# wwood/CoverM

Measured on NVIDIA H100. Metric: reads/sec `coverm contig` (mean+trimmed_mean+covered_fraction), higher is better.
Workload: dtype i32

## Files before the change

coverm_b200/csrc/cmb_k2.cuh:

```cuda
#pragma once
#include "cmb_k2_slots.cuh"

struct K2Args {
  const uint32_t* off_span;
  const uint32_t* len;
  const uint32_t* chunk_first;
  const int32_t* carry_in;
  cmb_contig_stats* rows;
  uint32_t tid_begin, n_local, n_chunks, excl;
  int32_t* arena;
  const uint32_t* word_off;
  const uint16_t* buckets;
  uint32_t* span_bits;
  uint32_t* load_stats;
  const uint64_t* bin_base;
  uint32_t* bins;
  uint64_t pool_cap;
  uint32_t* bin_hi;
  uint32_t* error_flags;
};

#ifndef CMB_K2_DENSE_SPANS
#define CMB_K2_DENSE_SPANS 160
#endif
constexpr uint32_t K2_DENSE_SPANS = CMB_K2_DENSE_SPANS;
static_assert(K2_STAGES >= 2, "a round's rows are requested one round before it is reduced");
static_assert(K2_CHUNK_SPANS == CHUNK_SPANS && K2_WARPS == 8, "a chunk is 8 bitmap words of 32 spans");

constexpr uint32_t K2_ROUND = 32;
constexpr uint32_t K2_BUF_BYTES = K2_ROUND * 128;
constexpr uint32_t K2_BOX_ROWS = K2_ROUND;
constexpr uint32_t K2_STAGE_CODES = 1024;
constexpr uint32_t K2_STAGE_BYTES = K2_STAGE_CODES * 2;
template <bool BUCKETS>
__host__ __device__ constexpr uint32_t k2_warp_bytes() { return BUCKETS ? K2_BUF_BYTES + K2_STAGES * K2_STAGE_BYTES : K2_STAGES * K2_BUF_BYTES; }
constexpr uint32_t K2_CHUNK_CONTIGS = 16;
struct K2ChunkContigs {
  uint64_t bin[K2_CHUNK_CONTIGS + 1];
  uint32_t start[K2_CHUNK_CONTIGS];
  uint32_t len[K2_CHUNK_CONTIGS];
};
struct K2WarpTables {
  K2ChunkContigs ct;
  uint8_t span[2][K2_CHUNK_SPANS];
  uint8_t pre[2][8];
};
static_assert(sizeof(K2WarpTables) % 8 == 0, "the contig tables hold u64 bins");
constexpr uint32_t K2_SMEM_MISC = K2_WARPS * K2_STAGES * 8  +
                                  K2_WARPS * 128  +
                                  K2_WARPS * sizeof(K2WarpTables);
template <bool BUCKETS>
__host__ __device__ constexpr uint32_t k2_smem_bytes() { return K2_WARPS * k2_warp_bytes<BUCKETS>() + K2_SMEM_MISC; }
static_assert(k2_warp_bytes<true>() % 1024 == 0 && k2_warp_bytes<false>() % 1024 == 0, "round buffers are whole swizzle atoms");

__device__ __forceinline__ uint32_t k2_rounds(uint32_t pop, bool dense) { return dense ? CHUNK_SPANS / K2_ROUND : (pop + K2_ROUND - 1) / K2_ROUND; }

template <bool HIST, bool CLEAN, bool BUCKETS>
__global__ void __launch_bounds__(K2_THREADS, CMB_K2_MINBLOCKS) k2_scan_reduce(const __grid_constant__ CUtensorMap tmap, const K2Args a) {
  extern __shared__ __align__(1024) uint8_t smem[];
  const uint32_t lane = threadIdx.x & 31, warp = threadIdx.x >> 5;
  constexpr uint32_t RING = K2_WARPS * k2_warp_bytes<BUCKETS>();
  uint8_t* ring = smem + warp * k2_warp_bytes<BUCKETS>();
  uint64_t* bars = reinterpret_cast<uint64_t*>(smem + RING) + warp * K2_STAGES;
  uint32_t* words = reinterpret_cast<uint32_t*>(smem + RING + K2_WARPS * K2_STAGES * 8) + warp * 32;
  uint32_t(&w)[8] = *reinterpret_cast<uint32_t(*)[8]>(words + 8);
  uint32_t* wo = words + 16;
  K2WarpTables& tb = reinterpret_cast<K2WarpTables*>(smem + RING + K2_WARPS * K2_STAGES * 8 + K2_WARPS * 128)[warp];

  const bool hist = HIST && __ldg(a.bin_base + a.n_local) <= a.pool_cap;
  if (HIST && !hist && blockIdx.x == 0 && threadIdx.x == 0) atomicOr(a.error_flags, ERR_CAPACITY);

  const uint32_t W = gridDim.x * K2_WARPS, g = blockIdx.x * K2_WARPS + warp;
  auto load_word = [&](uint32_t ck) -> uint32_t { return ck < a.n_chunks && lane < K2_WARPS ? a.span_bits[ck * K2_WARPS + lane] : 0u; };
  auto load_off = [&](uint32_t ck) -> uint32_t { return BUCKETS && ck < a.n_chunks && lane <= K2_WARPS ? __ldg(a.word_off + ck * K2_WARPS + lane) : 0u; };
  auto spread = [&](uint32_t word, uint32_t* to, uint32_t t, uint32_t off = 0, uint32_t* to_off = nullptr) -> uint32_t {
    __syncwarp();
    if (to && lane < K2_WARPS) to[lane] = word;
    if (to_off && lane <= K2_WARPS) to_off[lane] = off;
    const uint32_t pop = __reduce_add_sync(FULL, __popc(word));
    const uint32_t mw = pop >= K2_DENSE_SPANS && lane < K2_WARPS ? ~0u : word;
    uint32_t before = __popc(mw);
#pragma unroll
    for (uint32_t d = 1; d < K2_WARPS; d <<= 1) {
      const uint32_t o = __shfl_up_sync(FULL, before, d);
      if (lane >= d) before += o;
    }
    before -= __popc(mw);
    if (lane < K2_WARPS) tb.pre[t][lane] = (uint8_t)before;
    k2_span_table_lane(__shfl_sync(FULL, mw, lane / 4), __shfl_sync(FULL, before, lane / 4), lane, tb.span[t]);
    __syncwarp();
    return pop;
  };

  if (lane == 0) {
    for (uint32_t s = 0; s < K2_STAGES; ++s) mbar_init(smem_u32(bars + s), 1);
    fence_barrier_init();
  }
  if (BUCKETS)
    for (uint32_t u = lane; u < K2_BUF_BYTES / 16; u += 32) reinterpret_cast<int4*>(ring)[u] = make_int4(0, 0, 0, 0);
  __syncwarp();

  uint32_t fk = g, fr = 0, fns = 0;
  uint32_t f_word = load_word(fk);
  uint32_t f_off = load_off(fk), fo = 0;
  uint32_t n_loaded = 0, n_dense = 0, n_events = 0;
  auto f_enter = [&]() {
    for (; fk < a.n_chunks; fk += W) {
      const uint32_t word = f_word;
      f_word = load_word(fk + W);
      fo = f_off;
      f_off = load_off(fk + W);
      const uint32_t pop = spread(word, nullptr, 0);
      fns = pop >= K2_DENSE_SPANS ? CHUNK_SPANS : pop;
      fr = 0;
      if (fns) {
        n_loaded += fns;
        n_dense += pop >= K2_DENSE_SPANS;
        return;
      }
    }
  };
  auto fill = [&](uint32_t fi) {
    if (fk < a.n_chunks) {
      uint8_t* buf = ring + (fi % K2_STAGES) * K2_BUF_BYTES;
      const uint32_t bar = smem_u32(bars + fi % K2_STAGES);
      if constexpr (BUCKETS) {
        uint32_t wf, wl;
        k2_round_words(tb.span[0], fns, fr, wf, wl);
        const uint32_t b0 = __shfl_sync(FULL, fo, wf), b1 = __shfl_sync(FULL, fo, wl + 1);
        const uint32_t base = b0 & ~7u, units = min((b1 - base + 7) / 8, K2_STAGE_CODES / 8);
        uint8_t* stg = ring + K2_BUF_BYTES + (fi % K2_STAGES) * K2_STAGE_BYTES;
        const int4* src = reinterpret_cast<const int4*>(a.buckets + base);
        for (uint32_t u = lane; u < units; u += 32) cp_async_16(smem_u32(stg + u * 16), src + u);
        n_events += b1 - b0;
      } else if (fns >= K2_DENSE_SPANS) {
        if (lane == 0) {
          fence_proxy_async_smem();
          mbar_arrive_expect_tx(bar, K2_BUF_BYTES);
          tma_load_2d(smem_u32(buf), &tmap, 0, (int32_t)(fk * CHUNK_ROWS + fr * K2_BOX_ROWS), bar);
        }
      } else {
        const uint32_t n = min(K2_ROUND, fns - fr * K2_ROUND);
        const uint32_t jf = fr * K2_ROUND + lane, sp = jf < fns ? tb.span[0][jf] : 0u;
        const uint32_t q = lane >> 3, unit = lane & 7;
        const int4* src = reinterpret_cast<const int4*>(a.arena + (uint64_t)fk * CHUNK) + unit;
        for (uint32_t r0 = 0; r0 < n; r0 += 4) {
          const uint32_t row = r0 + q;
          const uint32_t rsp = __shfl_sync(FULL, sp, row & 31);
          if (row < n) cp_async_16(smem_u32(buf + row * 128 + ((unit ^ (row & 7)) << 4)), src + rsp * (SPAN / 4));
        }
        if (lane == 0) mbar_arrive(bar);
      }
      if (++fr == (fns + K2_ROUND - 1) / K2_ROUND) {
        fk += W;
        f_enter();
      }
    }
    cp_async_commit();
  };
  f_enter();
  for (uint32_t p = 0; p + 1 < K2_STAGES; ++p) fill(p);

  const uint32_t E = a.excl;
  auto flush = [&](uint32_t c, uint32_t sf, uint32_t sw, uint64_t sd, uint32_t top) {
    cmb_contig_stats* rowp = a.rows + a.tid_begin + c;
    if (sf) atomicAdd((unsigned long long*)&rowp->covered_full, (unsigned long long)sf);
    if (sw) atomicAdd((unsigned long long*)&rowp->covered_window, (unsigned long long)sw);
    if (sd) atomicAdd((unsigned long long*)&rowp->sum_depth_window, (unsigned long long)sd);
    if (top) atomicMax(a.bin_hi + c, top);
  };
  auto bin_add = [&](uint64_t bin0, uint64_t bin1, int depth, uint32_t cnt, uint32_t& top) {
    if (depth < 0 || (uint64_t)depth >= bin1 - bin0) {
      atomicOr(a.error_flags, ERR_INTERNAL);
      return;
    }
    atomicAdd(a.bins + bin0 + (uint32_t)depth, cnt);
    top = max(top, (uint32_t)depth);
  };

  uint32_t c_word = load_word(g), c_off = load_off(g);
  uint32_t n_cf = 0, n_cl = 0;
  int n_cin = 0;
  if (g < a.n_chunks) {
    n_cf = __ldg(a.chunk_first + g);
    n_cl = __ldg(a.chunk_first + g + 1);
    n_cin = __ldg(a.carry_in + g);
  }
  uint32_t i = 0;
  for (uint32_t k = g; k < a.n_chunks; k += W) {
    const uint32_t word = c_word, off = c_off, cf = n_cf, cl = n_cl;
    const int cin = n_cin;
    c_word = load_word(k + W);
    c_off = load_off(k + W);
    if (k + W < a.n_chunks) {
      n_cf = __ldg(a.chunk_first + k + W);
      n_cl = __ldg(a.chunk_first + k + W + 1);
      n_cin = __ldg(a.carry_in + k + W);
    }
    const bool tabled = BUCKETS && cl - cf < K2_CHUNK_CONTIGS;
    uint32_t t_start = 0, t_len = 0;
    uint64_t t_bin = 0;
    if (tabled && lane <= cl - cf) {
      t_start = __ldg(a.off_span + cf + lane);
      t_len = __ldg(a.len + cf + lane);
    }
    if (HIST && tabled && lane <= cl - cf + 1) t_bin = __ldg(a.bin_base + cf + lane);
    const uint32_t pop = spread(word, w, 1, off, BUCKETS ? wo : nullptr);
    if (tabled && lane <= cl - cf) {
      tb.ct.start[lane] = t_start;
      tb.ct.len[lane] = t_len;
    }
    if (HIST && tabled && lane <= cl - cf + 1) tb.ct.bin[lane] = t_bin;
    __syncwarp();
    const bool dense = pop >= K2_DENSE_SPANS;
    const uint32_t nr = k2_rounds(pop, dense), nslots = dense ? CHUNK_SPANS : pop;
    const uint32_t span0 = k * CHUNK_SPANS;
    uint32_t pc = cf, c_first = 0xffffffffu;
    int pd = cin;
    for (uint32_t r = 0; r < nr; ++r, ++i) {
      __syncwarp();
      fill(i + K2_STAGES - 1);
      const uint32_t j = r * K2_ROUND + lane;
      const bool valid = j < nslots;
      const uint32_t s = valid ? tb.span[1][j] : CHUNK_SPANS, sn = j + 1 < nslots ? tb.span[1][j + 1] : CHUNK_SPANS;
      uint32_t c = 0xffffffffu, cstart = 0;
      K2Win win{0u, 0u, 0u};
      uint64_t bin0 = 0, bin1 = 0;
      if (valid && tabled) {
        uint32_t t = 0;
#pragma unroll
        for (uint32_t h = K2_CHUNK_CONTIGS / 2; h; h >>= 1)
          if (t + h <= cl - cf && tb.ct.start[t + h] <= span0 + s) t += h;
        c = cf + t;
        cstart = tb.ct.start[t];
        win = k2_window(tb.ct.len[t], E);
        if (hist) {
          bin0 = tb.ct.bin[t];
          bin1 = tb.ct.bin[t + 1];
        }
      } else if (valid) {
        uint32_t lo = cf, hi = cl;
        while (lo < hi) {
          const uint32_t mid = (lo + hi + 1) >> 1;
          if (__ldg(a.off_span + mid) <= span0 + s) lo = mid;
          else hi = mid - 1;
        }
        c = lo;
        cstart = __ldg(a.off_span + c);
        win = k2_window(__ldg(a.len + c), E);
        if (hist) {
          bin0 = __ldg(a.bin_base + c);
          bin1 = __ldg(a.bin_base + c + 1);
        }
      }
      const uint32_t st = i % K2_STAGES;
      if (!BUCKETS) mbar_wait(smem_u32(bars + st), (i / K2_STAGES) & 1);
      cp_async_wait<K2_STAGES - 1>();
      __syncwarp();
      uint8_t* rows = BUCKETS ? ring : ring + st * K2_BUF_BYTES;
      if (BUCKETS) {
        const uint32_t wf = __shfl_sync(FULL, s, 0) / 32, wl = __shfl_sync(FULL, s, min(nslots - r * K2_ROUND, K2_ROUND) - 1) / 32;
        const uint32_t base = wo[wf] & ~7u;
        const uint16_t* stg = reinterpret_cast<const uint16_t*>(ring + K2_BUF_BYTES + st * K2_STAGE_BYTES);
        k2_round_events(
            w, tb.pre[1], wo, dense, r, wf, wl, lane, 32,
            [&](uint32_t p) { return p - base < K2_STAGE_CODES ? (uint32_t)stg[p - base] : (uint32_t)__ldg(a.buckets + p); },
            [&](uint32_t rw, uint32_t e, int d) {
              atomicAdd(reinterpret_cast<int*>(rows + rw * 128 + (((e >> 2) ^ (rw & 7)) << 4) + ((e & 3) << 2)), d);
            });
        __syncwarp();
      }
      uint8_t* row = rows + lane * 128;
      int total = 0;
      uint32_t ev = 0;
      if (valid) {
#pragma unroll
        for (uint32_t u = 0; u < SPAN / 4; ++u) {
          const int4 v = *reinterpret_cast<const int4*>(row + ((u ^ (lane & 7)) << 4));
          const uint32_t e4 = (v.x != 0 ? 1u : 0u) | (v.y != 0 ? 2u : 0u) | (v.z != 0 ? 4u : 0u) | (v.w != 0 ? 8u : 0u);
          total += (v.x + v.y) + (v.z + v.w);
          ev |= e4 << (4 * u);
          if constexpr (!BUCKETS && CLEAN)
            if (e4) reinterpret_cast<int4*>(a.arena + (uint64_t)(span0 + s) * SPAN)[u] = make_int4(0, 0, 0, 0);
        }
      }
      int incl = total;
#pragma unroll
      for (uint32_t d = 1; d < 32; d <<= 1) {
        const int ov = __shfl_up_sync(FULL, incl, d);
        const uint32_t oc = __shfl_up_sync(FULL, c, d);
        if (lane >= d && oc == c) incl += ov;
      }
      const int depth = incl - total + (c == pc ? pd : 0);
      const uint32_t rel = (span0 + s - cstart) * SPAN;
      const uint32_t from = j == 0 && c == cf ? (span0 - cstart) * SPAN : rel;
      const uint32_t to = rel + (sn - s) * SPAN;
      K2Acc acc{0u, 0u, 0ull};
      uint32_t top = 0;
      int out = 0;
      if (valid)
        out = k2_slot_runs(
            acc, win, depth, ev, rel, from, to,
            [&](uint32_t e) { return *reinterpret_cast<const int*>(row + (((e >> 2) ^ (lane & 7)) << 4) + ((e & 3) << 2)); },
            [&](int d, uint32_t n) {
              if (hist) bin_add(bin0, bin1, d, n, top);
            });
      if (BUCKETS)
#pragma unroll
        for (uint32_t u = 0; u < SPAN / 4; ++u)
          if (ev >> (4 * u) & 15u) *reinterpret_cast<int4*>(row + ((u ^ (lane & 7)) << 4)) = make_int4(0, 0, 0, 0);
      pc = __shfl_sync(FULL, c, 31);
      pd = __shfl_sync(FULL, out, 31);
      if (r == 0) c_first = __shfl_sync(FULL, c, 0);
      uint32_t sf = acc.cov_full, sw = acc.cov_win;
      uint64_t sd = acc.sum_win;
#pragma unroll
      for (uint32_t d = 1; d < 32; d <<= 1) {
        const uint32_t of = __shfl_down_sync(FULL, sf, d), ow = __shfl_down_sync(FULL, sw, d);
        const uint64_t od = __shfl_down_sync(FULL, sd, d);
        const uint32_t ot = HIST ? __shfl_down_sync(FULL, top, d) : 0u;
        const uint32_t oc = __shfl_down_sync(FULL, c, d);
        if (lane + d < 32 && oc == c) {
          sf += of;
          sw += ow;
          sd += od;
          top = max(top, ot);
        }
      }
      const uint32_t prev_c = __shfl_up_sync(FULL, c, 1);
      if (valid && (lane == 0 || prev_c != c)) flush(c, sf, sw, sd, top);
    }
    if (lane == 0 && cin != 0 && c_first != cf) {
      const uint32_t cstart = tabled ? tb.ct.start[0] : __ldg(a.off_span + cf);
      const K2Win win = k2_window(tabled ? tb.ct.len[0] : __ldg(a.len + cf), E);
      const uint32_t s0 = nslots ? tb.span[1][0] : CHUNK_SPANS;
      K2Acc acc{0u, 0u, 0ull};
      uint32_t top = 0;
      const uint32_t nw = k2_close_run(acc, win, cin, (span0 - cstart) * SPAN, (span0 + s0 - cstart) * SPAN);
      if (hist && nw)
        bin_add(tabled ? tb.ct.bin[0] : __ldg(a.bin_base + cf), tabled ? tb.ct.bin[1] : __ldg(a.bin_base + cf + 1), cin, nw, top);
      flush(cf, acc.cov_full, acc.cov_win, acc.sum_win, top);
    }
    if (CLEAN && word) a.span_bits[k * K2_WARPS + lane] = 0;
  }
  if (lane == 0 && n_loaded) {
    atomicAdd(a.load_stats + 0, n_loaded);
    atomicAdd(a.load_stats + 1, n_dense);
    if (BUCKETS) atomicAdd(a.load_stats + 2, n_events);
  }
}
```

coverm_b200/csrc/cmb_k2_slots.cuh:

```cuda
#pragma once
#include <stdint.h>

#ifdef __CUDACC__
#define K2_HD __host__ __device__ __forceinline__
#else
#define K2_HD inline
#endif

constexpr uint32_t K2_CHUNK_SPANS = 256;

K2_HD uint32_t k2_popc(uint32_t x) {
#ifdef __CUDA_ARCH__
  return __popc(x);
#else
  return (uint32_t)__builtin_popcount(x);
#endif
}

K2_HD uint32_t k2_low_bit(uint32_t x) {
#ifdef __CUDA_ARCH__
  return (uint32_t)__ffs((int)x) - 1u;
#else
  return (uint32_t)__builtin_ctz(x);
#endif
}

K2_HD uint32_t k2_nth_bit(uint32_t x, uint32_t n) {
  uint32_t pos = 0;
#pragma unroll
  for (uint32_t w = 16; w; w >>= 1) {
    const uint32_t lo = k2_popc(x & ((1u << w) - 1u));
    if (n >= lo) {
      n -= lo;
      x >>= w;
      pos += w;
    }
  }
  return pos;
}

K2_HD uint32_t k2_slot_span(const uint32_t (&w)[8], uint32_t j, bool dense) {
  if (dense) return j < K2_CHUNK_SPANS ? j : K2_CHUNK_SPANS;
  uint32_t base = 0, word = 0, rem = j;
  bool found = false;
#pragma unroll
  for (uint32_t q = 0; q < 8; ++q) {
    const uint32_t p = k2_popc(w[q]);
    if (!found) {
      if (rem < p) {
        found = true;
        base = 32 * q;
        word = w[q];
      } else {
        rem -= p;
      }
    }
  }
  return found ? base + k2_nth_bit(word, rem) : K2_CHUNK_SPANS;
}

K2_HD void k2_span_table_lane(uint32_t word, uint32_t before, uint32_t lane, uint8_t* span) {
  const uint32_t q = lane / 4, sh = (lane % 4) * 8;
  uint32_t m = (word >> sh) & 255u, j = before + k2_popc(word & ((1u << sh) - 1u));
  while (m) {
    span[j++] = (uint8_t)(32 * q + sh + k2_low_bit(m));
    m &= m - 1;
  }
}


K2_HD void k2_round_words(const uint32_t (&w)[8], uint32_t nslots, bool dense, uint32_t r, uint32_t& wf, uint32_t& wl) {
  const uint32_t j1 = r * 32 + 31 < nslots ? r * 32 + 31 : nslots - 1;
  wf = k2_slot_span(w, r * 32, dense) / 32;
  wl = k2_slot_span(w, j1, dense) / 32;
}
K2_HD void k2_round_words(const uint8_t* span, uint32_t nslots, uint32_t r, uint32_t& wf, uint32_t& wl) {
  const uint32_t j1 = r * 32 + 31 < nslots ? r * 32 + 31 : nslots - 1;
  wf = span[r * 32] / 32u;
  wl = span[j1] / 32u;
}

K2_HD uint32_t k2_bucket_row(const uint32_t (&w)[8], bool dense, uint32_t r, uint32_t q, uint32_t before, uint32_t code) {
  const uint32_t b = (code & 1023u) / 32u;
  if (dense) return q * 32 + b - r * 32;
  return before + k2_popc(w[q] & ((1u << b) - 1u)) - r * 32;
}

template <class Code, class Add>
K2_HD void k2_round_events(const uint32_t (&w)[8], const uint8_t* pre, const uint32_t* wo, bool dense, uint32_t r, uint32_t wf,
                           uint32_t wl, uint32_t p0, uint32_t step, Code code, Add add) {
  uint32_t q = wf, before = pre[wf];
  const uint32_t p1 = wo[wl + 1];
  for (uint32_t p = wo[wf] + p0; p < p1; p += step) {
    while (q < wl && wo[q + 1] <= p) before = pre[++q];
    const uint32_t c = code(p);
    const uint32_t row = k2_bucket_row(w, dense, r, q, before, c);
    if (row < 32) add(row, c & 31u, (c >> 10) & 1u ? -1 : 1);
  }
}
template <class Code, class Add>
K2_HD void k2_round_events(const uint32_t (&w)[8], const uint32_t* wo, bool dense, uint32_t r, uint32_t wf, uint32_t wl,
                           uint32_t p0, uint32_t step, Code code, Add add) {
  uint8_t pre[8];
  for (uint32_t q = 0, before = 0; q < 8; before += k2_popc(w[q++])) pre[q] = (uint8_t)before;
  k2_round_events(w, pre, wo, dense, r, wf, wl, p0, step, code, add);
}

struct K2Win {
  uint32_t L, w0, w1;
};
K2_HD K2Win k2_window(uint32_t L, uint32_t E) {
  K2Win w{L, 0u, 0u};
  if (2ull * E < L) {
    w.w0 = E;
    w.w1 = L - E;
  }
  return w;
}

struct K2Acc {
  uint32_t cov_full, cov_win;
  uint64_t sum_win;
};

K2_HD uint32_t k2_close_run(K2Acc& a, const K2Win& w, int depth, uint32_t from, uint32_t to) {
  const uint32_t nc = (to < w.L ? to : w.L) - (from < w.L ? from : w.L);
  const uint32_t t1 = to < w.w0 ? w.w0 : (to > w.w1 ? w.w1 : to), f1 = from < w.w0 ? w.w0 : (from > w.w1 ? w.w1 : from);
  const uint32_t nw = t1 - f1;
  if (depth > 0) {
    a.cov_full += nc;
    a.cov_win += nw;
  }
  a.sum_win += (uint64_t)(int64_t)depth * nw;
  return nw;
}

template <class Delta, class Hist>
K2_HD int k2_slot_runs(K2Acc& a, const K2Win& w, int depth, uint32_t ev, uint32_t rel, uint32_t from, uint32_t to, Delta delta,
                       Hist hist) {
  while (ev) {
    const uint32_t j = k2_low_bit(ev);
    ev &= ev - 1;
    const uint32_t nw = k2_close_run(a, w, depth, from, rel + j);
    if (nw && depth != 0) hist(depth, nw);
    depth += delta(j);
    from = rel + j;
  }
  const uint32_t nw = k2_close_run(a, w, depth, from, to);
  if (nw && depth != 0) hist(depth, nw);
  return depth;
}
```

Measured before the change: 5.364 billion.

## Track touched positions with per-row bitmasks instead of scanning full smem rows

In the bucketed path, each event scatter now also sets a bit in a per-row shared-memory mask. The row total and event set are then computed from that mask instead of reading all 32 words of the row. Delta reads clear the word in place, replacing the separate int4 zeroing pass, and the row swizzle changes to a rotate-by-row word index. This cuts shared-memory traffic on sparse rows at the cost of an extra shared atomicOr per event, and it also skips zero-net events inside the run walk.

Measured after the change: 5.591 billion, median of 6. 1.04x the previous value.

```diff
diff --git a/coverm_b200/csrc/cmb_k2.cuh b/coverm_b200/csrc/cmb_k2.cuh
--- a/coverm_b200/csrc/cmb_k2.cuh
+++ b/coverm_b200/csrc/cmb_k2.cuh
@@ -49,8 +49,9 @@
 constexpr uint32_t K2_SMEM_MISC = K2_WARPS * K2_STAGES * 8  +
                                   K2_WARPS * 128  +
                                   K2_WARPS * sizeof(K2WarpTables);
+constexpr uint32_t K2_MASK_BYTES = K2_ROUND * 4;
 template <bool BUCKETS>
-__host__ __device__ constexpr uint32_t k2_smem_bytes() { return K2_WARPS * k2_warp_bytes<BUCKETS>() + K2_SMEM_MISC; }
+__host__ __device__ constexpr uint32_t k2_smem_bytes() { return K2_WARPS * k2_warp_bytes<BUCKETS>() + K2_SMEM_MISC + (BUCKETS ? K2_WARPS * K2_MASK_BYTES : 0); }
 static_assert(k2_warp_bytes<true>() % 1024 == 0 && k2_warp_bytes<false>() % 1024 == 0, "round buffers are whole swizzle atoms");
 
 __device__ __forceinline__ uint32_t k2_rounds(uint32_t pop, bool dense) { return dense ? CHUNK_SPANS / K2_ROUND : (pop + K2_ROUND - 1) / K2_ROUND; }
@@ -66,6 +67,7 @@
   uint32_t(&w)[8] = *reinterpret_cast<uint32_t(*)[8]>(words + 8);
   uint32_t* wo = words + 16;
   K2WarpTables& tb = reinterpret_cast<K2WarpTables*>(smem + RING + K2_WARPS * K2_STAGES * 8 + K2_WARPS * 128)[warp];
+  uint32_t* masks = reinterpret_cast<uint32_t*>(smem + RING + K2_SMEM_MISC) + warp * K2_ROUND;
 
   const bool hist = HIST && __ldg(a.bin_base + a.n_local) <= a.pool_cap;
   if (HIST && !hist && blockIdx.x == 0 && threadIdx.x == 0) atomicOr(a.error_flags, ERR_CAPACITY);
@@ -96,8 +98,10 @@
     for (uint32_t s = 0; s < K2_STAGES; ++s) mbar_init(smem_u32(bars + s), 1);
     fence_barrier_init();
   }
-  if (BUCKETS)
+  if (BUCKETS) {
     for (uint32_t u = lane; u < K2_BUF_BYTES / 16; u += 32) reinterpret_cast<int4*>(ring)[u] = make_int4(0, 0, 0, 0);
+    masks[lane] = 0;
+  }
   __syncwarp();
 
   uint32_t fk = g, fr = 0, fns = 0;
@@ -266,14 +270,19 @@
             w, tb.pre[1], wo, dense, r, wf, wl, lane, 32,
             [&](uint32_t p) { return p - base < K2_STAGE_CODES ? (uint32_t)stg[p - base] : (uint32_t)__ldg(a.buckets + p); },
             [&](uint32_t rw, uint32_t e, int d) {
-              atomicAdd(reinterpret_cast<int*>(rows + rw * 128 + (((e >> 2) ^ (rw & 7)) << 4) + ((e & 3) << 2)), d);
+              atomicAdd(reinterpret_cast<int*>(rows) + k2_row_word(rw, e), d);
+              atomicOr(masks + rw, 1u << e);
             });
         __syncwarp();
       }
       uint8_t* row = rows + lane * 128;
+      int* const rowi = reinterpret_cast<int*>(rows);
       int total = 0;
       uint32_t ev = 0;
-      if (valid) {
+      if (BUCKETS) {
+        ev = masks[lane];
+        total = k2_mask_total(ev, [&](uint32_t e) { return rowi[k2_row_word(lane, e)]; });
+      } else if (valid) {
 #pragma unroll
         for (uint32_t u = 0; u < SPAN / 4; ++u) {
           const int4 v = *reinterpret_cast<const int4*>(row + ((u ^ (lane & 7)) << 4));
@@ -301,14 +310,20 @@
       if (valid)
         out = k2_slot_runs(
             acc, win, depth, ev, rel, from, to,
-            [&](uint32_t e) { return *reinterpret_cast<const int*>(row + (((e >> 2) ^ (lane & 7)) << 4) + ((e & 3) << 2)); },
+            [&](uint32_t e) {
+              if constexpr (BUCKETS) {
+                int* p = rowi + k2_row_word(lane, e);
+                const int d = *p;
+                *p = 0;
+                return d;
+              } else {
+                return *reinterpret_cast<const int*>(row + (((e >> 2) ^ (lane & 7)) << 4) + ((e & 3) << 2));
+              }
+            },
             [&](int d, uint32_t n) {
               if (hist) bin_add(bin0, bin1, d, n, top);
             });
-      if (BUCKETS)
-#pragma unroll
-        for (uint32_t u = 0; u < SPAN / 4; ++u)
-          if (ev >> (4 * u) & 15u) *reinterpret_cast<int4*>(row + ((u ^ (lane & 7)) << 4)) = make_int4(0, 0, 0, 0);
+      if (BUCKETS && ev) masks[lane] = 0;
       pc = __shfl_sync(FULL, c, 31);
       pd = __shfl_sync(FULL, out, 31);
       if (r == 0) c_first = __shfl_sync(FULL, c, 0);
diff --git a/coverm_b200/csrc/cmb_k2_slots.cuh b/coverm_b200/csrc/cmb_k2_slots.cuh
--- a/coverm_b200/csrc/cmb_k2_slots.cuh
+++ b/coverm_b200/csrc/cmb_k2_slots.cuh
@@ -98,6 +98,8 @@
     if (row < 32) add(row, c & 31u, (c >> 10) & 1u ? -1 : 1);
   }
 }
+K2_HD uint32_t k2_row_word(uint32_t row, uint32_t e) { return row * 32u + ((row + e) & 31u); }
+
 template <class Code, class Add>
 K2_HD void k2_round_events(const uint32_t (&w)[8], const uint32_t* wo, bool dense, uint32_t r, uint32_t wf, uint32_t wl,
                            uint32_t p0, uint32_t step, Code code, Add add) {
@@ -135,15 +137,24 @@
   return nw;
 }
 
+template <class Delta>
+K2_HD int k2_mask_total(uint32_t ev, Delta delta) {
+  int total = 0;
+  for (; ev; ev &= ev - 1) total += delta(k2_low_bit(ev));
+  return total;
+}
+
 template <class Delta, class Hist>
 K2_HD int k2_slot_runs(K2Acc& a, const K2Win& w, int depth, uint32_t ev, uint32_t rel, uint32_t from, uint32_t to, Delta delta,
                        Hist hist) {
   while (ev) {
     const uint32_t j = k2_low_bit(ev);
     ev &= ev - 1;
+    const int d = delta(j);
+    if (d == 0) continue;
     const uint32_t nw = k2_close_run(a, w, depth, from, rel + j);
     if (nw && depth != 0) hist(depth, nw);
-    depth += delta(j);
+    depth += d;
     from = rel + j;
   }
   const uint32_t nw = k2_close_run(a, w, depth, from, to);
```
